# chinmay5/vit_ae_plus_plus

Measured on AMD Instinct MI355X. Metric: pretrain volumes/sec (96^3x4ch, mask 0.75) at 1/2/4/8 MI355X + recon-loss parity, higher is better.
Workload: dtype bf16; 1 GPU; ViT-B/16^3 contrastive MAE full optimisation step (fwd+loss+bwd+grad-norm+AdamW), synthetic BraTS-shape 96^3x4ch, batch 4/GPU, mask 0.75 (BASELINE config 2); global_batch=4, parallelism=dp1, rccl_ranks=1, hip_graph=True, weights=product initialize_weights, seed 0

## Files before the change

### vit_ae_plus_plus_amd/csrc/gemm_bt.hip

```cpp
#include "gemm_bt.hpp"

namespace vglds {

template <int BM, int BN, int WM, int WN, bool A_KC, bool B_KC>
__device__ __forceinline__ void gemm_bt_body(const GArgs& p, const int bid, const int zid, unsigned char* smem) {
    using Cf = BtCfg<BM, BN, WM, WN>;
    constexpr int NW = Cf::NW, HM = Cf::HM, HN = Cf::HN, FM = Cf::FM, FN = Cf::FN, NF = FM * FN;
    constexpr int A_HALF = Cf::A_HALF, B_HALF = Cf::B_HALF, BUF = Cf::BUF;
    constexpr bool STAGGER = NW == 8;
    constexpr int PA = pieces<HM, A_KC, NW>(), PB = pieces<HN, B_KC, NW>();
    constexpr int NACC = NF == 1 ? 2 : 1;
    constexpr bool ASM_READS = !A_KC || !B_KC;
    const int T = p.tiles_m * p.tiles_n;
    const int xq = T >> 3, xr = T & 7, xcd = bid & 7;
    const int lin = (xcd < xr ? xcd * (xq + 1) : xr * (xq + 1) + (xcd - xr) * xq) + (bid >> 3);
    if ((bid >> 3) >= xq + (xcd < xr ? 1 : 0)) return;
    const int tn = p.xcd_m ? lin % p.tiles_n : lin / p.tiles_m;
    const int tm = p.xcd_m ? lin / p.tiles_n : lin % p.tiles_m;
    const int m0 = tm * BM, n0 = tn * BN;
    const int kbeg = zid * p.k_per_split;
    const int nk = (min(p.K, kbeg + p.k_per_split) - kbeg) / BK;
    const int lane = threadIdx.x & 63;
    const int wave = __builtin_amdgcn_readfirstlane(threadIdx.x >> 6);
    const int wm = wave / WN, wn = wave % WN;
// ... 171 lines not shown
template <int BM, int BN, int WM, int WN>
static void bt_launch_cfg(const GArgs& p, bool a_kc, bool b_kc, hipStream_t st) {
    const dim3 grid(8 * cdiv((long)p.tiles_m * p.tiles_n, 8), 1, p.splits), block(64 * WM * WN);
    if (a_kc && b_kc) hipLaunchKernelGGL((gemm_bt_kernel<BM, BN, WM, WN, true, true>), grid, block, 0, st, p);
    else if (a_kc && !b_kc) hipLaunchKernelGGL((gemm_bt_kernel<BM, BN, WM, WN, true, false>), grid, block, 0, st, p);
    else if (!a_kc && !b_kc) hipLaunchKernelGGL((gemm_bt_kernel<BM, BN, WM, WN, false, false>), grid, block, 0, st, p);
}

bool bt_tile_dims(int id, int& bm, int& bn) {
    switch (id) {
        case 0: bm = 256; bn = 256; return true;
        case 3: bm = 128; bn = 128; return true;
        case 4: bm = 128; bn = 128; return true;
        case 5: bm = 64; bn = 64; return true;
        case 6: bm = 128; bn = 256; return true;
        default: return false;
    }
}

int bt_launch(GArgs p, int a_kc, int b_kc, int id, hipStream_t st) {
    int bm, bn;
    if (!bt_tile_dims(id, bm, bn)) return VITAE_ERR_INVALID_ARG;
    if (!p.vec_epi || p.a_rowsum || (p.K % BK) || p.splits < 1) return VITAE_ERR_UNSUPPORTED_SHAPE;
    if (!a_kc && b_kc) return VITAE_ERR_UNSUPPORTED_SHAPE;
    if (!bt_k_ranges(p.K, 2, p.splits, p.k_per_split)) return VITAE_ERR_UNSUPPORTED_SHAPE;
    p.tiles_m = cdiv(p.M, bm); p.tiles_n = cdiv(p.N, bn);
    if (p.splits > 1 && (!p.ws || id == 0 || (long)p.tiles_m * p.tiles_n > VITAE_GLDS_TICKETS || p.epi == VITAE_EPI_GELU)) return VITAE_ERR_UNSUPPORTED_SHAPE;
    if (id == 6 && (a_kc || b_kc)) return VITAE_ERR_UNSUPPORTED_SHAPE;
    if (id == 0) bt_launch_cfg<256, 256, 2, 4>(p, a_kc, b_kc, st);
    else if (id == 4 || id == 6) ws_launch(p, a_kc, b_kc, id, st);
    else if (id == 5) ws64_launch(p, a_kc, b_kc, st);
    else bt_launch_cfg<128, 128, 2, 2>(p, a_kc, b_kc, st);
    return vitae_launch_status();
}

int bt_wgrad_group_launch(GArgs* ps, int n, int splits, hipStream_t st, int kind ) {
    if (n < 1 || n > 4) return VITAE_ERR_INVALID_ARG;
    BtGroup g;
    int total = 0, tiles = 0;
    const int K = ps[0].K;
    int kps;
    if (!bt_k_ranges(K, 2, splits, kps)) return VITAE_ERR_UNSUPPORTED_SHAPE;
    for (int i = 0; i < 4; ++i) {
        g.start[i] = total;
        if (i >= n) { g.p[i] = g.p[0]; continue; }
        GArgs& p = ps[i];
// ... 18 lines not shown
```

### vit_ae_plus_plus_amd/csrc/gemm_bt.hpp

```cpp
#pragma once
#include <cstdlib>
#include <type_traits>
#include "glds_gemm.hpp"

namespace vglds {

using K0 = std::integral_constant<int, 0>; using K1 = std::integral_constant<int, 1>;
using K2 = std::integral_constant<int, 2>; using K3 = std::integral_constant<int, 3>;

__device__ __forceinline__ void wg_barrier() {
    __builtin_amdgcn_sched_barrier(0);
    __builtin_amdgcn_s_barrier();
    __builtin_amdgcn_sched_barrier(0);
}


template <int S, int PT> __device__ __forceinline__ void wait_tiles(const int fly) {
    if (S >= 5 && fly >= 3) wait_vmcnt<(S >= 5 ? 3 : 1) * PT>();
    else if (S >= 4 && fly >= 2) wait_vmcnt<(S >= 4 ? 2 : 1) * PT>();
    else if (fly >= 1) wait_vmcnt<PT>();
    else wait_vmcnt<0>();
}

static inline bool bt_k_ranges(const int K, const int min_tiles, int& splits, int& kps) {
// ... 372 lines not shown
        __builtin_amdgcn_sched_barrier(0);
        asm volatile("s_waitcnt lgkmcnt(0)" ::: "memory");
        if (t + 1 < nk) {
            wg_barrier();
            stage = stage + 1 == S ? 0 : stage + 1;
            const unsigned char* TN = smem + stage * STG;
            rd(TN, K0{}); rd(TN, K1{});
            __builtin_amdgcn_sched_barrier(0);
        }
        mm(K2{}); mm(K3{});
    }
}

void ws_launch(const GArgs& p, int a_kc, int b_kc, int id , hipStream_t st);
void ws_wgrad_group_launch(const BtGroup& g, int total, int splits, int kind , hipStream_t st);
void ws64_launch(const GArgs& p, int a_kc, int b_kc, hipStream_t st);

}
```

### vit_ae_plus_plus_amd/csrc/gemm_glds.hip

```cpp
#include <cstdlib>
#include "common.hpp"
#include "glds_tiles.hpp"
#include "glds_gemm.hpp"
#include "vitae_hip.h"

namespace {

using namespace vglds;

long long* g_gemm_dbg = nullptr;
double* g_wgrad_sqacc = nullptr;
int g_wgrad_sq_mask = 0, g_wgrad_sq_stride = 0;
static inline void set_sq(vglds::GArgs& p) { p.sqacc = g_wgrad_sqacc; p.sq_mask = g_wgrad_sq_mask; p.sq_stride = g_wgrad_sq_stride; }

struct EpiPre { f32x4 bias, res[4]; bool have; };

template <int BM, int BN, int NW>
__device__ __forceinline__ void epilogue_prefetch(const GArgs& p, int m0, int n0, EpiPre& e) {
    constexpr int NT = 64 * NW, CG = BN / 4, RPP = NT / CG, PASSES = BM / RPP;
    e.have = false;
    if constexpr (BM == 64 && BN == 64 && NW == 4) {
        static_assert(PASSES == 4, "prefetch geometry");
        if (!p.vec_epi) return;
        e.have = true;
// ... 528 lines not shown
    const int nkt = K / BK;
    static const int ws_on = getenv("VITAE_BT_WS") ? atoi(getenv("VITAE_BT_WS")) : 1;
    static const double ws_kt = getenv("VITAE_BT_WS_KT") ? atof(getenv("VITAE_BT_WS_KT")) : 800.0;
    static const int ws_min_rows = getenv("VITAE_BT_WS_MIN_ROWS") ? atoi(getenv("VITAE_BT_WS_MIN_ROWS")) : 2048;
    static const int ws_min_rows_fwd = getenv("VITAE_BT_WS_MIN_ROWS_FWD") ? atoi(getenv("VITAE_BT_WS_MIN_ROWS_FWD")) : 800;
    static const int ws_long_k = getenv("VITAE_BT_WS_LONG_K") ? atoi(getenv("VITAE_BT_WS_LONG_K")) : 8192;
    static const double ws_kt_w = getenv("VITAE_BT_WS_KT_W") ? atof(getenv("VITAE_BT_WS_KT_W")) : 900.0;
    static const double ws_fix = getenv("VITAE_BT_WS_FIX") ? atof(getenv("VITAE_BT_WS_FIX")) : 14000.0;
    static const int ws64_on = getenv("VITAE_BT_WS64") ? atoi(getenv("VITAE_BT_WS64")) : 1;
    static const double ws64_kt_w = getenv("VITAE_BT_WS64_KT_W") ? atof(getenv("VITAE_BT_WS64_KT_W")) : 650.0;
    static const int ws_long_any = getenv("VITAE_BT_WS_LONG_ANY") ? atoi(getenv("VITAE_BT_WS_LONG_ANY")) : 1;
    static const double bt_fix0 = getenv("VITAE_BT_FIX0") ? atof(getenv("VITAE_BT_FIX0")) : 9000.0;
    static const double bt_fix1 = getenv("VITAE_BT_FIX1") ? atof(getenv("VITAE_BT_FIX1")) : 4000.0;
    static const double wsw_kt = getenv("VITAE_BT_WSW_KT") ? atof(getenv("VITAE_BT_WSW_KT")) : 1350.0;
    static const int wsw_on = getenv("VITAE_BT_WSW") ? atoi(getenv("VITAE_BT_WSW")) : 1;
    for (int id : {0, 3, 4, 5, 6}) {
        if (only >= 0 && id != only) continue;
        if (id == 6 && (a_kc || b_kc || (g_bt_mode < 0 && !wsw_on))) continue;
        if (id == 5 && g_bt_mode != 5 && (!ws64_on || !allow_ws64)) continue;
        if (g_bt_mode >= 0 && id != g_bt_mode) continue;
        if (id == 4 && g_bt_mode < 0 && !ws_on) continue;
        if (id == 4 && g_bt_mode < 0 && (a_kc ? M : K) < ((a_kc && b_kc) ? ws_min_rows_fwd : ws_min_rows) && !(K >= ws_long_k && (ws_long_any || (a_kc ? M : K) < 1024))) continue;
        if (id == 6 && g_bt_mode < 0 && K < ws_min_rows && K < ws_long_k && (long)M * N < (1L << 22)) continue;
        int bm, bn;
        bt_tile_dims(id, bm, bn);
        const bool forced = g_bt_mode >= 0;
        if (!forced && (M < bm / 2 || N < bn / 2)) continue;
        const long tiles = (long)cdiv(M, bm) * cdiv(N, bn);
        static const int fsplit = getenv("VITAE_BT_SPLIT") ? atoi(getenv("VITAE_BT_SPLIT")) : 0;
        for (int s = 1; s <= (id >= 3 && allow_split ? (id == 6 ? 4 : 8) : 1); ++s) {
            if (forced && fsplit > 0 && s != fsplit) continue;
            const int kps = cdiv(cdiv(K, s), BK) * BK;
            if (cdiv(K, kps) != s || kps < (forced ? 2 : 4) * BK || K - (s - 1) * kps < 2 * BK) continue;
            if (s > 1 && (tiles > VITAE_GLDS_TICKETS || (cap >= 0 && VITAE_GLDS_TICKETS + tiles * s * bm * bn > cap))) continue;
            const double wgs = (double)tiles * s, slots = id == 3 ? 512 : 256;
            const double rounds = (double)cdiv((long)wgs, (long)slots);
            const double nk = (double)nkt / s;
            const double per = id == 0 ? 3000 + ((!a_kc && !b_kc) ? 4300 : 2950) * nk + 14500
                             : id == 6 ? ws_fix + 4000 + wsw_kt * nk + (s > 1 ? 9000 + 4000 * s : 0)
                             : id == 4 ? ws_fix + ((!a_kc && !b_kc) ? ws_kt_w : ws_kt) * nk + (s > 1 ? 6000 + 2200 * s : 0)
                                       : 4500 + 1800 * nk + 7500 + (s > 1 ? bt_fix0 + bt_fix1 * s : 0);
            double clk = rounds * per;
            if (id == 5) {
                const double over = wgs > 256 ? (wgs - 256) / 256 : 0, kt64 = (!a_kc && !b_kc && wgs >= 512) ? ws64_kt_w : 420;
                const double lat = (6500 + kt64 * nk + (s > 1 ? 3000 + 1000 * s : 0)) * (1 + 0.2 * over), thr = wgs * (3000 + kt64 * nk) / 256;
                clk = lat > thr ? lat : thr;
                if (nkt >= 128) clk *= 1.25;
            }
            if (clk < best.clocks) best = BtPlan{id, s, clk};
        }
    }
    if (best.tile < 0 || g_bt_mode >= 0 || only >= 0) return best;
    if (best.clocks >= 0.92 * est_64row(M, N, K, allow_split, !a_kc && !b_kc) * (nkt >= 128 ? 1.25 : 1.0)) return BtPlan{-1, 1, 0.0};
    return best;
}

template <int BM1, int BN1>
void launch_pair(int id2, dim3 grid, hipStream_t st, const GArgs& p1, const GArgs& p2, int nb1) {
    dim3 block(256);
    if (id2 == 0) hipLaunchKernelGGL((gemm_glds_pair_kernel<BM1, BN1, 64, 64>), grid, block, 0, st, p1, p2, nb1);
    else hipLaunchKernelGGL((gemm_glds_pair_kernel<BM1, BN1, 64, 128>), grid, block, 0, st, p1, p2, nb1);
}

}

extern "C" int vitae_gemm_glds_set_bt_tile(int mode) {
    if (mode < -2 || mode > 6 || mode == 1 || mode == 2) return VITAE_ERR_INVALID_ARG;
    g_bt_mode = mode;
    return VITAE_OK;
}

extern "C" int vitae_gemm_glds_bt_choice(int a_kcontig, int b_kcontig, int M, int N, int K) { return bt_plan(M, N, K, a_kcontig, b_kcontig, true).tile; }

extern "C" int vitae_gemm_glds_pick_split_k(int M, int N, int K) {
    const BtPlan bp = bt_plan(M, N, K, 1, 1, true);
    if (bp.tile >= 0) return bp.split;
    return old_split_rule(M, N, K);
}

extern "C" int vitae_gemm_glds_pick_split_k_form(int a_kcontig, int b_kcontig, int M, int N, int K) {
    const BtPlan bp = bt_plan(M, N, K, a_kcontig, b_kcontig, true);
    if (bp.tile >= 0) return bp.split;
// ... 36 lines not shown
    p.C = C; p.ldc = ldc; p.C16 = reinterpret_cast<__bf16*>(C16); p.ldc16 = ldc16;
    p.M = M; p.N = N; p.K = K;
    int kps = cdiv(cdiv(K, split_k), BK) * BK;
    split_k = cdiv(K, kps);
    if (split_k > 1 && !splitk_ws) return VITAE_ERR_INVALID_ARG;
    p.k_per_split = kps; p.splits = split_k;
    p.bias = bias; p.residual = residual; p.ldr = ldr; p.aux = aux; p.ldaux = ldaux;
    p.epi = epi; p.aux16 = aux16; p.auxd = auxd; p.accumulate = accumulate; p.ws = splitk_ws; p.out_colsum = out_colsum_accum; p.a_rowsum = nullptr;
    p.dbg = g_gemm_dbg;
    const Tile t = pick_tile(M, N);
    p.tiles_m = cdiv(M, t.bm); p.tiles_n = cdiv(N, t.bn);
    p.xcd_m = xcd_by_rows(M, N);
    p.vec_epi = vec_epilogue_ok(p);
    if (!a_kcontig && !b_kcontig) set_sq(p);
    if (p.vec_epi) {
        const BtPlan bp = forced ? *forced : bt_plan(M, N, K, a_kcontig, b_kcontig, epi != VITAE_EPI_GELU);
        if (bp.tile >= 0 && bp.split == split_k) {
            p.splits = split_k;
            return bt_launch(p, a_kcontig, b_kcontig, bp.tile, (hipStream_t)stream);
        }
    }
    if (split_k > 1 && (long)p.tiles_m * p.tiles_n > VITAE_GLDS_TICKETS) return VITAE_ERR_UNSUPPORTED_SHAPE;
    dim3 grid(glds_blocks(p), 1, split_k);
    hipStream_t st = (hipStream_t)stream;
    static const int pipe_max = getenv("VITAE_GLDS_PIPE_MAX_WGS") ? atoi(getenv("VITAE_GLDS_PIPE_MAX_WGS")) : 512;
    if (t.id == 0 && a_kcontig && b_kcontig && (long)grid.x * split_k <= pipe_max) {
        hipLaunchKernelGGL(gemm_glds_pipe_kernel, grid, dim3(256), 0, st, p);
        return vitae_launch_status();
    }
    if (t.id == 1) launch<64, 128>(p, a_kcontig != 0, b_kcontig != 0, grid, st);
    else launch<64, 64>(p, a_kcontig != 0, b_kcontig != 0, grid, st);
// ... 121 lines not shown
    const int epi_flags = (aux16 ? VITAE_EPI_AUX_BF16 : 0) | (auxd ? VITAE_EPI_AUX_DERIV : 0);
    if (dx_accumulate && !dx) return VITAE_ERR_INVALID_ARG;
    if ((N % BK) || (Mpad % BK) || (K & 7) || Mpad < M) return VITAE_ERR_UNSUPPORTED_SHAPE;
    if ((long)(M > N ? M : N) * K >= (1L << 31)) return VITAE_ERR_UNSUPPORTED_SHAPE;
    if ((long)Mpad * N >= (1L << 30) || (long)Mpad * K >= (1L << 30) || (long)N * K >= (1L << 30)) return VITAE_ERR_UNSUPPORTED_SHAPE;
    const long cap = splitk_ws && splitk_ws_floats > 0 ? splitk_ws_floats : 0;
    if (split_k > 1 && vitae_gemm_glds_ws_floats(M, K, split_k) > cap) return VITAE_ERR_INVALID_ARG;
    if (((uintptr_t)dy16 & 15) || ((uintptr_t)w16 & 15) || ((uintptr_t)x16 & 15)) return VITAE_ERR_UNSUPPORTED_SHAPE;
    if (!dw) {
        const BtPlan pd = bt_plan(M, K, N, 1, 0, true, cap);
        int sp = pd.tile >= 0 ? pd.split : old_split_rule(M, K, N);
        while (pd.tile < 0 && sp > 1 && vitae_gemm_glds_ws_floats(M, K, sp) > cap) --sp;
        return gemm_glds_launch(1, 0, dy16, N, w16, K, dx, K, dx16, K, M, K, N, nullptr, nullptr, 0, epi | epi_flags,
                                aux, K, dx_accumulate, sp, splitk_ws, dx_colsum_accum, stream, &pd);
    }
    auto ws64_pair = [&](int split) -> int {
        GArgs p1, p2;
        p1.A = reinterpret_cast<const __bf16*>(dy16); p1.lda = N;
        p1.B = reinterpret_cast<const __bf16*>(w16); p1.ldb = K;
        p1.C = dx; p1.ldc = K; p1.C16 = reinterpret_cast<__bf16*>(dx16); p1.ldc16 = K;
        p1.M = M; p1.N = K; p1.K = N; p1.k_per_split = N; p1.splits = split;
        p1.bias = nullptr; p1.residual = nullptr; p1.ldr = 0; p1.aux = aux; p1.ldaux = K; p1.epi = epi; p1.aux16 = aux16; p1.auxd = auxd;
        p1.accumulate = dx_accumulate != 0; p1.ws = splitk_ws; p1.out_colsum = dx_colsum_accum; p1.a_rowsum = nullptr; p1.dbg = g_gemm_dbg;
        p1.xcd_m = xcd_by_rows(M, K); p1.tiles_m = 0; p1.tiles_n = 0;
        p1.vec_epi = vec_epilogue_ok(p1);
        p2.A = reinterpret_cast<const __bf16*>(dy16); p2.lda = N;
        p2.B = reinterpret_cast<const __bf16*>(x16); p2.ldb = K;
        p2.C = dw; p2.ldc = K; p2.C16 = reinterpret_cast<__bf16*>(dw16); p2.ldc16 = K;
        p2.M = N; p2.N = K; p2.K = Mpad; p2.k_per_split = Mpad; p2.splits = 1;
        p2.bias = nullptr; p2.residual = nullptr; p2.ldr = 0; p2.aux = nullptr; p2.ldaux = 0; p2.epi = VITAE_EPI_NONE;
        p2.accumulate = dw_accumulate; p2.ws = nullptr; p2.out_colsum = nullptr; p2.a_rowsum = dy_colsum_accum; p2.dbg = g_gemm_dbg;
        set_sq(p2);
        p2.xcd_m = xcd_by_rows(N, K); p2.tiles_m = 0; p2.tiles_n = 0;
        p2.vec_epi = vec_epilogue_ok(p2);
        if (!p1.vec_epi || !p2.vec_epi) return VITAE_ERR_UNSUPPORTED_SHAPE;
        const char* wsq_env = getenv("VITAE_WS64Q");
        const int wsq = wsq_env ? atoi(wsq_env) : 0;
        const int rc = wsq ? ws64q_pair_launch(p1, p2, (hipStream_t)stream) : VITAE_ERR_UNSUPPORTED_SHAPE;
        return rc != VITAE_ERR_UNSUPPORTED_SHAPE ? rc : ws64_pair_launch(p1, p2, (hipStream_t)stream);
    };
    if (g_bt_mode == -1 || g_bt_mode == 5) {
        const BtPlan pd = bt_plan(M, K, N, 1, 0, true, cap), pw = bt_plan(N, K, Mpad, 0, 0, false, cap);
        if (pd.tile == 5 && pw.tile == 5) {
            const int rc = ws64_pair(pd.split);
            if (rc != VITAE_ERR_UNSUPPORTED_SHAPE) return rc;
        }
    }
    if (g_bt_mode != -2) {
        const BtPlan pd = bt_plan(M, K, N, 1, 0, true, cap, false), pw = bt_plan(N, K, Mpad, 0, 0, true, cap, false);
        if (pd.tile >= 0 || pw.tile >= 0) {
            auto fit = [&](const BtPlan& bp, int m, int n, int k) {
                if (bp.tile >= 0) return bp.split;
                int sp = old_split_rule(m, n, k);
                while (sp > 1 && vitae_gemm_glds_ws_floats(m, n, sp) > cap) --sp;
                return sp;
            };
            int rc = gemm_glds_launch(1, 0, dy16, N, w16, K, dx, K, dx16, K, M, K, N, nullptr, nullptr, 0, epi | epi_flags,
                                      aux, K, dx_accumulate, fit(pd, M, K, N), splitk_ws, dx_colsum_accum, stream, &pd);
            if (rc != VITAE_OK) return rc;
// ... 135 lines not shown
```

### vit_ae_plus_plus_amd/csrc/gemm_ws64.hip

```cpp
#include "gemm_bt.hpp"

namespace vglds {

#ifndef VITAE_WS64_STAGES
#define VITAE_WS64_STAGES 4
#endif
constexpr int WS64_SMEM = VITAE_WS64_STAGES * 16384;
template <bool A_KC, bool B_KC, int S, bool RS, bool W2 = false>
__device__ __forceinline__ void gemm_ws64_body(const GArgs& p, const WsHot& h, const int bid, const int zid, unsigned char* smem) {
#ifndef VITAE_WS64_PRODUCERS
#define VITAE_WS64_PRODUCERS 4
#endif
    constexpr int BM = 64, BN = 64, NWC = 4, NWP = VITAE_WS64_PRODUCERS;
    constexpr int A_T = BM * BK * 2, B_T = BN * BK * 2, STG = A_T + (W2 ? 2 : 1) * B_T;
    constexpr int PA = pieces<BM, A_KC, NWP>(), PB = pieces<BN, B_KC, NWP>(), PT = PA + (W2 ? 2 : 1) * PB;
    static_assert(!W2 || (A_KC && B_KC && !RS), "two weight planes: the forward form");
    static_assert(S >= 3 && S <= 5 && (S - 2) * PT <= 63, "stage count");
    const int T = h.tiles_m * h.tiles_n;
    const int xq = T >> 3, xr = T & 7, xcd = bid & 7;
    const int lin = (xcd < xr ? xcd * (xq + 1) : xr * (xq + 1) + (xcd - xr) * xq) + (bid >> 3);
    if ((bid >> 3) >= xq + (xcd < xr ? 1 : 0)) return;
    const int tn = (h.xcd_m & 1) ? lin % h.tiles_n : lin / h.tiles_m;
    const int tm = (h.xcd_m & 1) ? lin / h.tiles_n : lin % h.tiles_m;
    const int m0 = tm * BM, n0 = tn * BN;
    const int kbeg = zid * h.kps;
    const int nk = (min(h.K, kbeg + h.kps) - kbeg) / BK;
    const int lane = threadIdx.x & 63;
    const int wave = __builtin_amdgcn_readfirstlane(threadIdx.x >> 6);
// ... 36 lines not shown
    }
    const int wm = wave >> 1, wn = wave & 1;
    const int l31 = lane & 31, hi = lane >> 5;
    f32x16 acc[2];
#pragma unroll
    for (int h = 0; h < 2; ++h)
#pragma unroll
        for (int i = 0; i < 16; ++i) acc[h][i] = 0.f;
    const bool rowsum = RS && p.a_rowsum != nullptr && tn == 0 && wn == 0;
    f32x16 accx;
#pragma unroll
    for (int i = 0; i < 16; ++i) accx[i] = 0.f;
    bf16x8 ones;
#pragma unroll
    for (int i = 0; i < 8; ++i) ones[i] = (__bf16)1.0f;
    bf16x8 fa[BK / 16], fb[BK / 16], fb2[W2 ? BK / 16 : 1];
    constexpr int RK = (A_KC ? 1 : 2) + (W2 ? 2 : 1) * (B_KC ? 1 : 2);
    auto rd = [&](const unsigned char* TA, auto kk_c) {
        constexpr int kk = decltype(kk_c)::value;
        fa[kk] = frag_asm<BM, A_KC>(TA, wm * 32, kk, lane);
        fb[kk] = frag_asm<BN, B_KC>(TA + A_T, wn * 32, kk, lane);
        if constexpr (W2) fb2[kk] = frag_asm<BN, B_KC>(TA + A_T + B_T, wn * 32, kk, lane);
    };
    auto mm = [&](auto kk_c) {
        constexpr int kk = decltype(kk_c)::value;
        frag_tie(fa[kk]); frag_tie(fb[kk]);
        if constexpr (W2) {
            frag_tie(fb2[kk]);
            acc[kk & 1] = __builtin_amdgcn_mfma_f32_32x32x16_bf16(fa[kk], fb2[kk], acc[kk & 1], 0, 0, 0);
        }
        acc[kk & 1] = __builtin_amdgcn_mfma_f32_32x32x16_bf16(fa[kk], fb[kk], acc[kk & 1], 0, 0, 0);
        if constexpr (RS) {
            if (rowsum) accx = __builtin_amdgcn_mfma_f32_32x32x16_bf16(fa[kk], ones, accx, 0, 0, 0);
        }
    };
    const int nq = n0 + wn * 32 + 4 * (lane % 8);
    f32x4 bias4 = {0.f, 0.f, 0.f, 0.f};
    if (p.bias && nq < p.N) bias4 = *reinterpret_cast<const f32x4*>(p.bias + nq);
    stamp(0);
    wg_barrier();
    stamp(1);
    ws64_consume<2 * RK, S, STG>(smem, nk, rd, mm);
    if (RS && rowsum && l31 == 0) {
#pragma unroll
        for (int r = 0; r < 16; ++r) {
            const int m = m0 + wm * 32 + crow(r, hi);
            if (m < p.M) atomicAdd(p.a_rowsum + m, accx[r]);
        }
    }
    stamp(2);
    f32x16 accs[1][1];
#pragma unroll
    for (int i = 0; i < 16; ++i) accs[0][0][i] = acc[0][i] + acc[1][i];
    __syncthreads();
    float* Tw = reinterpret_cast<float*>(smem) + wave * 1024;
    if (p.splits > 1) {
        const int tile = p.tile0 + tm * p.tiles_n + tn;
        float* part = p.ws + VITAE_GLDS_TICKETS + (long)tile * p.splits * (BM * BN);
        const __amdgpu_buffer_rsrc_t rs = __builtin_amdgcn_make_buffer_rsrc(part, 0, p.splits * (BM * BN * 4), 0x00020000);
        typedef unsigned u32x4 __attribute__((ext_vector_type(4)));
        const int toff = (int)threadIdx.x * 16;
#pragma unroll
        for (int g = 0; g < 4; ++g) {
            const f32x4 v = {accs[0][0][4 * g], accs[0][0][4 * g + 1], accs[0][0][4 * g + 2], accs[0][0][4 * g + 3]};
            __builtin_amdgcn_raw_buffer_store_b128(__builtin_bit_cast(u32x4, v), rs, (zid * 4 + g) * (256 * 16) + toff, 0, 16);
        }
        asm volatile("s_waitcnt vmcnt(0)" ::: "memory");
        __syncthreads();
        int* flag = reinterpret_cast<int*>(smem + 4 * 4096);
        if (threadIdx.x == 0) *flag = __hip_atomic_fetch_add(reinterpret_cast<int*>(p.ws) + tile, 1, __ATOMIC_RELAXED, __HIP_MEMORY_SCOPE_AGENT);
        __syncthreads();
        stamp(3);
        if (*flag != p.splits - 1) return;
#pragma unroll
        for (int i = 0; i < 16; ++i) accs[0][0][i] = 0.f;
#pragma unroll 1
        for (int sp0 = 0; sp0 < p.splits; sp0 += 4) {
            f32x4 v[4][4];
#pragma unroll
            for (int u = 0; u < 4; ++u) {
                const int sp = min(sp0 + u, p.splits - 1);
#pragma unroll
                for (int g = 0; g < 4; ++g)
                    v[u][g] = __builtin_bit_cast(f32x4, __builtin_amdgcn_raw_buffer_load_b128(rs, (sp * 4 + g) * (256 * 16) + toff, 0, 16));
            }
#pragma unroll
            for (int u = 0; u < 4; ++u)
                if (sp0 + u < p.splits) {
#pragma unroll
                    for (int g = 0; g < 4; ++g)
#pragma unroll
                        for (int e = 0; e < 4; ++e) accs[0][0][4 * g + e] += v[u][g][e];
                }
        }
        if (threadIdx.x == 0) __hip_atomic_store(reinterpret_cast<int*>(p.ws) + tile, 0, __ATOMIC_RELAXED, __HIP_MEMORY_SCOPE_AGENT);
    }
    stamp(4);
    bt_park_quadrant<1, 1, 1>(accs, lane, Tw);
    __builtin_amdgcn_wave_barrier();
    float sqs = 0.f;
    { f32x4 cz = {0.f, 0.f, 0.f, 0.f}; bt_wave_epilogue<1, 1>(p, bt_epilogue_kind(p), m0 + wm * 32, n0 + wn * 32, Tw, lane, sqs, bias4, cz, false); }
    stamp(5);
    if (p.sqacc) {
        sqs = wave_sum(sqs);
        float* red = reinterpret_cast<float*>(smem + 4 * 4096 + 64);
        if (lane == 0) red[wave] = sqs;
        __syncthreads();
        if (threadIdx.x == 0) atomicAdd(sq_slot(p), (double)((red[0] + red[1]) + (red[2] + red[3])));
    }
    if (p.dbg) { asm volatile("s_waitcnt vmcnt(0)" ::: "memory"); stamp(6); }
}

template <bool A_KC, bool B_KC>
__global__ __launch_bounds__(64 * (4 + VITAE_WS64_PRODUCERS), 2) void gemm_ws64_kernel(WS_HOT_PARAMS, const GArgs p) {
    __shared__ __attribute__((aligned(1024))) unsigned char smem[WS64_SMEM];
    const WsHot h = WS_HOT_FROM_PARAMS;
    gemm_ws64_body<A_KC, B_KC, VITAE_WS64_STAGES, false>(p, h, blockIdx.x, blockIdx.z, smem);
}

void ws64_launch(const GArgs& p, int a_kc, int b_kc, hipStream_t st) {
    const dim3 grid(8 * cdiv((long)p.tiles_m * p.tiles_n, 8), 1, p.splits), block(64 * (4 + VITAE_WS64_PRODUCERS));
    if (a_kc && b_kc) hipLaunchKernelGGL((gemm_ws64_kernel<true, true>), grid, block, 0, st, WS_HOT_ARGS(p), p);
    else if (a_kc && !b_kc) hipLaunchKernelGGL((gemm_ws64_kernel<true, false>), grid, block, 0, st, WS_HOT_ARGS(p), p);
    else hipLaunchKernelGGL((gemm_ws64_kernel<false, false>), grid, block, 0, st, WS_HOT_ARGS(p), p);
}

constexpr int WS64W2_STAGES = 3;
__global__ __launch_bounds__(64 * (4 + VITAE_WS64_PRODUCERS), 2) void gemm_ws64_w2_kernel(WS_HOT_PARAMS, const GArgs p) {
    __shared__ __attribute__((aligned(1024))) unsigned char smem[WS64W2_STAGES * 24576];
    gemm_ws64_body<true, true, WS64W2_STAGES, false, true>(p, WS_HOT_FROM_PARAMS, blockIdx.x, blockIdx.z, smem);
}

int ws64_w2_launch(GArgs p, hipStream_t st) {
    if (!p.vec_epi || !p.B2 || p.a_rowsum || (p.K % BK) || p.splits < 1) return VITAE_ERR_UNSUPPORTED_SHAPE;
    if (!bt_k_ranges(p.K, 2, p.splits, p.k_per_split)) return VITAE_ERR_UNSUPPORTED_SHAPE;
    p.tiles_m = cdiv(p.M, 64); p.tiles_n = cdiv(p.N, 64); p.tile0 = 0;
    if (p.splits > 1 && (!p.ws || (long)p.tiles_m * p.tiles_n > VITAE_GLDS_TICKETS || p.epi == VITAE_EPI_GELU)) return VITAE_ERR_UNSUPPORTED_SHAPE;
    const dim3 grid(8 * cdiv((long)p.tiles_m * p.tiles_n, 8), 1, p.splits), block(64 * (4 + VITAE_WS64_PRODUCERS));
    hipLaunchKernelGGL(gemm_ws64_w2_kernel, grid, block, 0, st, WS_HOT_ARGS(p), p);
    return vitae_launch_status();
}

template <bool RS>
__global__ __launch_bounds__(64 * (4 + VITAE_WS64_PRODUCERS), 2) void gemm_ws64_pair_kernel(const __bf16* A, const __bf16* B1, const __bf16* B2, int lda, int ldb,
                                                                                           int M1, int N1, int K1, int K2, int kps1, int packed,
                                                                                           const GArgs p1, const GArgs p2) {
    __shared__ __attribute__((aligned(1024))) unsigned char smem[WS64_SMEM];
    const int nb1 = packed & 0xfffff, splits1 = (packed >> 20) & 15, dbg2 = (packed >> 25) & 2;
    if ((int)blockIdx.x < nb1 * splits1) {
        const WsHot h{A, B1, nullptr, lda, ldb, M1, N1, K1, (M1 + 63) >> 6, (N1 + 63) >> 6, ((packed >> 24) & 1) | dbg2, kps1};
        gemm_ws64_body<true, false, VITAE_WS64_STAGES, false>(p1, h, blockIdx.x % nb1, blockIdx.x / nb1, smem);
    } else {
        const WsHot h{A, B2, nullptr, lda, ldb, K1, N1, K2, (K1 + 63) >> 6, (N1 + 63) >> 6, ((packed >> 25) & 1) | dbg2, K2};
        gemm_ws64_body<false, false, VITAE_WS64_STAGES, RS>(p2, h, blockIdx.x - nb1 * splits1, 0, smem);
    }
}

int ws64_pair_launch(GArgs p1, GArgs p2, hipStream_t st) {
    if (!p1.vec_epi || !p2.vec_epi || (p1.K % BK) || (p2.K % BK) || p2.K < 2 * BK || p1.a_rowsum) return VITAE_ERR_UNSUPPORTED_SHAPE;
    if (p1.splits < 1) p1.splits = 1;
    if (!bt_k_ranges(p1.K, 2, p1.splits, p1.k_per_split)) return VITAE_ERR_UNSUPPORTED_SHAPE;
    p1.tiles_m = cdiv(p1.M, 64); p1.tiles_n = cdiv(p1.N, 64); p1.tile0 = 0;
    p2.tiles_m = cdiv(p2.M, 64); p2.tiles_n = cdiv(p2.N, 64); p2.tile0 = 0;
    p2.k_per_split = p2.K; p2.splits = 1;
    if (p1.splits > 1 && (!p1.ws || (long)p1.tiles_m * p1.tiles_n > VITAE_GLDS_TICKETS)) return VITAE_ERR_UNSUPPORTED_SHAPE;
    const int nb1 = 8 * cdiv((long)p1.tiles_m * p1.tiles_n, 8), nb2 = 8 * cdiv((long)p2.tiles_m * p2.tiles_n, 8);
    const dim3 grid(nb1 * p1.splits + nb2), block(64 * (4 + VITAE_WS64_PRODUCERS));
    if (p1.A != p2.A || p1.lda != p2.lda || p1.ldb != p2.ldb || p2.M != p1.K || p2.N != p1.N || nb1 >= (1 << 20) || p1.splits > 15 ||
        p1.lda >= (1L << 31) || p1.ldb >= (1L << 31)) return VITAE_ERR_UNSUPPORTED_SHAPE;
    const int packed = nb1 | p1.splits << 20 | (p1.xcd_m & 1) << 24 | (p2.xcd_m & 1) << 25 | ((p1.dbg || p2.dbg) ? 1 << 26 : 0);
    if (p2.a_rowsum) hipLaunchKernelGGL((gemm_ws64_pair_kernel<true>), grid, block, 0, st, p1.A, p1.B, p2.B, (int)p1.lda, (int)p1.ldb, p1.M, p1.N, p1.K,
                                        p2.K, p1.k_per_split, packed, p1, p2);
    else hipLaunchKernelGGL((gemm_ws64_pair_kernel<false>), grid, block, 0, st, p1.A, p1.B, p2.B, (int)p1.lda, (int)p1.ldb, p1.M, p1.N, p1.K,
                            p2.K, p1.k_per_split, packed, p1, p2);
    return vitae_launch_status();
}

}
```

### vit_ae_plus_plus_amd/csrc/glds_gemm.hpp

```cpp
#pragma once
#include "common.hpp"
#include "glds_tiles.hpp"
#include "vitae_hip.h"

namespace vglds {

struct GArgs {
    const __bf16* A; long lda;
    const __bf16* B; long ldb;
    float* C; long ldc;
    __bf16* C16; long ldc16;
    int M, N, K;
    int k_per_split, splits;
    const float* bias;
    const float* residual; long ldr;
    float* aux; long ldaux;
    int epi, accumulate;
    float* ws;
    float* out_colsum;
    float* a_rowsum;
    int vec_epi;
    int tiles_m, tiles_n;
    double* sqacc = nullptr;
    int sq_mask = 0, sq_stride = 0;
// ... 64 lines not shown
                if (acc_c) x += co[q];
                p.C[m * ldc + n] = x;
            }
            if (p.C16) p.C16[m * ldc16 + n] = (__bf16)x;
            csum += x;
            sqsum += x * x;
        }
        asm volatile("" ::: "memory");
    }
    return csum;
}

bool bt_tile_dims(int id, int& bm, int& bn);
int bt_launch(GArgs p, int a_kc, int b_kc, int id, hipStream_t st);
int bt_wgrad_group_launch(GArgs* ps, int n, int splits, hipStream_t st, int kind);
int ws64_pair_launch(GArgs p1, GArgs p2, hipStream_t st);
int ws64q_pair_launch(GArgs p1, GArgs p2, hipStream_t st);
int wsx3_launch(GArgs p, int a_kc, int b_kc, hipStream_t st);
int ws64_w2_launch(GArgs p, hipStream_t st);
int wsx3_slots();

}
```

Before: 1145 volumes/s.

## Add 128x64 warp-specialized tile variant and use it in backward dgrad/wgrad pair

Generalizes the warp-specialized 64x64 GEMM body to a 128-row tile (two A fragments sharing one B fragment, three pipeline stages) and adds it as tile id 7. By default, the fused backward dgrad+wgrad pair kernel switches to 128-row tiles when the tile count is high and the reduction depth is short. The aim is more MFMA work per B-fragment load and fewer workgroups, cutting LDS and global traffic per flop. In exchange the kernel uses more registers and shared memory and has fewer stages, which may hurt latency hiding or occupancy.

```diff
diff --git a/vit_ae_plus_plus_amd/csrc/gemm_bt.hip b/vit_ae_plus_plus_amd/csrc/gemm_bt.hip
--- a/vit_ae_plus_plus_amd/csrc/gemm_bt.hip
+++ b/vit_ae_plus_plus_amd/csrc/gemm_bt.hip
@@ -209,6 +209,7 @@
         case 4: bm = 128; bn = 128; return true;
         case 5: bm = 64; bn = 64; return true;
         case 6: bm = 128; bn = 256; return true;
+        case 7: bm = 128; bn = 64; return true;
         default: return false;
     }
 }
@@ -224,7 +225,7 @@
     if (id == 6 && (a_kc || b_kc)) return VITAE_ERR_UNSUPPORTED_SHAPE;
     if (id == 0) bt_launch_cfg<256, 256, 2, 4>(p, a_kc, b_kc, st);
     else if (id == 4 || id == 6) ws_launch(p, a_kc, b_kc, id, st);
-    else if (id == 5) ws64_launch(p, a_kc, b_kc, st);
+    else if (id == 5 || id == 7) ws64_launch(p, a_kc, b_kc, id, st);
     else bt_launch_cfg<128, 128, 2, 2>(p, a_kc, b_kc, st);
     return vitae_launch_status();
 }
diff --git a/vit_ae_plus_plus_amd/csrc/gemm_bt.hpp b/vit_ae_plus_plus_amd/csrc/gemm_bt.hpp
--- a/vit_ae_plus_plus_amd/csrc/gemm_bt.hpp
+++ b/vit_ae_plus_plus_amd/csrc/gemm_bt.hpp
@@ -410,6 +410,6 @@
 
 void ws_launch(const GArgs& p, int a_kc, int b_kc, int id , hipStream_t st);
 void ws_wgrad_group_launch(const BtGroup& g, int total, int splits, int kind , hipStream_t st);
-void ws64_launch(const GArgs& p, int a_kc, int b_kc, hipStream_t st);
-
-}
+void ws64_launch(const GArgs& p, int a_kc, int b_kc, int id , hipStream_t st);
+
+}
diff --git a/vit_ae_plus_plus_amd/csrc/gemm_glds.hip b/vit_ae_plus_plus_amd/csrc/gemm_glds.hip
--- a/vit_ae_plus_plus_amd/csrc/gemm_glds.hip
+++ b/vit_ae_plus_plus_amd/csrc/gemm_glds.hip
@@ -566,8 +566,9 @@
     static const double bt_fix1 = getenv("VITAE_BT_FIX1") ? atof(getenv("VITAE_BT_FIX1")) : 4000.0;
     static const double wsw_kt = getenv("VITAE_BT_WSW_KT") ? atof(getenv("VITAE_BT_WSW_KT")) : 1350.0;
     static const int wsw_on = getenv("VITAE_BT_WSW") ? atoi(getenv("VITAE_BT_WSW")) : 1;
-    for (int id : {0, 3, 4, 5, 6}) {
+    for (int id : {0, 3, 4, 5, 6, 7}) {
         if (only >= 0 && id != only) continue;
+        if (id == 7 && g_bt_mode != 7 && only != 7) continue;
         if (id == 6 && (a_kc || b_kc || (g_bt_mode < 0 && !wsw_on))) continue;
         if (id == 5 && g_bt_mode != 5 && (!ws64_on || !allow_ws64)) continue;
         if (g_bt_mode >= 0 && id != g_bt_mode) continue;
@@ -593,6 +594,12 @@
                              : id == 4 ? ws_fix + ((!a_kc && !b_kc) ? ws_kt_w : ws_kt) * nk + (s > 1 ? 6000 + 2200 * s : 0)
                                        : 4500 + 1800 * nk + 7500 + (s > 1 ? bt_fix0 + bt_fix1 * s : 0);
             double clk = rounds * per;
+            if (id == 7) {
+                const double over = wgs > 256 ? (wgs - 256) / 256 : 0, kt = ((!a_kc && !b_kc && wgs >= 512) ? ws64_kt_w : 420) * 1.5;
+                const double lat = (7500 + kt * nk + (s > 1 ? 3000 + 1000 * s : 0)) * (1 + 0.2 * over), thr = wgs * (4000 + kt * nk) / 256;
+                clk = lat > thr ? lat : thr;
+                if (nkt >= 128) clk *= 1.25;
+            }
             if (id == 5) {
                 const double over = wgs > 256 ? (wgs - 256) / 256 : 0, kt64 = (!a_kc && !b_kc && wgs >= 512) ? ws64_kt_w : 420;
                 const double lat = (6500 + kt64 * nk + (s > 1 ? 3000 + 1000 * s : 0)) * (1 + 0.2 * over), thr = wgs * (3000 + kt64 * nk) / 256;
@@ -617,7 +624,7 @@
 }
 
 extern "C" int vitae_gemm_glds_set_bt_tile(int mode) {
-    if (mode < -2 || mode > 6 || mode == 1 || mode == 2) return VITAE_ERR_INVALID_ARG;
+    if (mode < -2 || mode > 7 || mode == 1 || mode == 2) return VITAE_ERR_INVALID_ARG;
     g_bt_mode = mode;
     return VITAE_OK;
 }
@@ -684,7 +691,8 @@
     p.vec_epi = vec_epilogue_ok(p);
     if (!a_kcontig && !b_kcontig) set_sq(p);
     if (p.vec_epi) {
-        const BtPlan bp = forced ? *forced : bt_plan(M, N, K, a_kcontig, b_kcontig, epi != VITAE_EPI_GELU);
+        BtPlan bp = forced ? *forced : bt_plan(M, N, K, a_kcontig, b_kcontig, epi != VITAE_EPI_GELU);
+        if (!forced && g_bt_mode == 7 && bp.tile == 7) bp.split = split_k;
         if (bp.tile >= 0 && bp.split == split_k) {
             p.splits = split_k;
             return bt_launch(p, a_kcontig, b_kcontig, bp.tile, (hipStream_t)stream);
@@ -836,7 +844,7 @@
         return gemm_glds_launch(1, 0, dy16, N, w16, K, dx, K, dx16, K, M, K, N, nullptr, nullptr, 0, epi | epi_flags,
                                 aux, K, dx_accumulate, sp, splitk_ws, dx_colsum_accum, stream, &pd);
     }
-    auto ws64_pair = [&](int split) -> int {
+    auto ws64_pair = [&](int split, int bm1 = 64, int bm2 = 64) -> int {
         GArgs p1, p2;
         p1.A = reinterpret_cast<const __bf16*>(dy16); p1.lda = N;
         p1.B = reinterpret_cast<const __bf16*>(w16); p1.ldb = K;
@@ -858,13 +866,31 @@
         if (!p1.vec_epi || !p2.vec_epi) return VITAE_ERR_UNSUPPORTED_SHAPE;
         const char* wsq_env = getenv("VITAE_WS64Q");
         const int wsq = wsq_env ? atoi(wsq_env) : 0;
-        const int rc = wsq ? ws64q_pair_launch(p1, p2, (hipStream_t)stream) : VITAE_ERR_UNSUPPORTED_SHAPE;
-        return rc != VITAE_ERR_UNSUPPORTED_SHAPE ? rc : ws64_pair_launch(p1, p2, (hipStream_t)stream);
+        const int rc = (wsq && bm1 == 64 && bm2 == 64) ? ws64q_pair_launch(p1, p2, (hipStream_t)stream) : VITAE_ERR_UNSUPPORTED_SHAPE;
+        return rc != VITAE_ERR_UNSUPPORTED_SHAPE ? rc : ws64_pair_launch(p1, p2, (hipStream_t)stream, bm1, bm2);
     };
+    if (g_bt_mode == 7) {
+        const char* pt = getenv("VITAE_PAIR_TILES");
+        const int bm1 = (pt && pt[0] == '5') ? 64 : 128, bm2 = (pt && pt[0] && pt[1] == '5') ? 64 : 128;
+        const BtPlan pd = bt_plan(M, K, N, 1, 0, true, cap);
+        if (pd.tile == 7) {
+            const int rc = ws64_pair(pd.split, bm1, bm2);
+            if (rc != VITAE_ERR_UNSUPPORTED_SHAPE) return rc;
+        }
+    }
     if (g_bt_mode == -1 || g_bt_mode == 5) {
         const BtPlan pd = bt_plan(M, K, N, 1, 0, true, cap), pw = bt_plan(N, K, Mpad, 0, 0, false, cap);
         if (pd.tile == 5 && pw.tile == 5) {
-            const int rc = ws64_pair(pd.split);
+            static const int t7_on = getenv("VITAE_PAIR_T7") ? atoi(getenv("VITAE_PAIR_T7")) : 1;
+            int bm1 = 64, bm2 = 64;
+            if (g_bt_mode == -1 && t7_on && pd.split == 1) {
+                const long w5 = (long)cdiv(N, 64) * cdiv(K, 64), d5 = (long)cdiv(M, 64) * cdiv(K, 64);
+                if (N / BK <= 16 && d5 + (w5 >= 384 ? (long)cdiv(N, 128) * cdiv(K, 64) : w5) >= 448) {
+                    bm1 = 128;
+                    if (w5 >= 384) bm2 = 128;
+                }
+            }
+            const int rc = ws64_pair(pd.split, bm1, bm2);
             if (rc != VITAE_ERR_UNSUPPORTED_SHAPE) return rc;
         }
     }
diff --git a/vit_ae_plus_plus_amd/csrc/gemm_ws64.hip b/vit_ae_plus_plus_amd/csrc/gemm_ws64.hip
--- a/vit_ae_plus_plus_amd/csrc/gemm_ws64.hip
+++ b/vit_ae_plus_plus_amd/csrc/gemm_ws64.hip
@@ -6,12 +6,13 @@
 #define VITAE_WS64_STAGES 4
 #endif
 constexpr int WS64_SMEM = VITAE_WS64_STAGES * 16384;
-template <bool A_KC, bool B_KC, int S, bool RS, bool W2 = false>
+template <bool A_KC, bool B_KC, int S, bool RS, bool W2 = false, int BM = 64>
 __device__ __forceinline__ void gemm_ws64_body(const GArgs& p, const WsHot& h, const int bid, const int zid, unsigned char* smem) {
 #ifndef VITAE_WS64_PRODUCERS
 #define VITAE_WS64_PRODUCERS 4
 #endif
-    constexpr int BM = 64, BN = 64, NWC = 4, NWP = VITAE_WS64_PRODUCERS;
+    constexpr int BN = 64, NWC = 4, NWP = VITAE_WS64_PRODUCERS, FM = BM / 64;
+    static_assert(BM == 64 || (BM == 128 && !W2), "64 or 128 rows");
     constexpr int A_T = BM * BK * 2, B_T = BN * BK * 2, STG = A_T + (W2 ? 2 : 1) * B_T;
     constexpr int PA = pieces<BM, A_KC, NWP>(), PB = pieces<BN, B_KC, NWP>(), PT = PA + (W2 ? 2 : 1) * PB;
     static_assert(!W2 || (A_KC && B_KC && !RS), "two weight planes: the forward form");
@@ -78,24 +79,46 @@
     bf16x8 ones;
 #pragma unroll
     for (int i = 0; i < 8; ++i) ones[i] = (__bf16)1.0f;
-    bf16x8 fa[BK / 16], fb[BK / 16], fb2[W2 ? BK / 16 : 1];
-    constexpr int RK = (A_KC ? 1 : 2) + (W2 ? 2 : 1) * (B_KC ? 1 : 2);
+    bf16x8 fa[FM][BK / 16], fb[BK / 16], fb2[W2 ? BK / 16 : 1];
+    constexpr int RK = FM * (A_KC ? 1 : 2) + (W2 ? 2 : 1) * (B_KC ? 1 : 2);
+    static_assert(2 * RK <= 15, "the counted lgkmcnt of ws64_consume");
+    bf16x8 sel[2];
+    if constexpr (FM == 2 && RS) {
+#pragma unroll
+        for (int i = 0; i < 8; ++i) {
+            sel[0][i] = (__bf16)((lane & 16) ? 0.0f : 1.0f);
+            sel[1][i] = (__bf16)((lane & 16) ? 1.0f : 0.0f);
+        }
+    }
     auto rd = [&](const unsigned char* TA, auto kk_c) {
         constexpr int kk = decltype(kk_c)::value;
-        fa[kk] = frag_asm<BM, A_KC>(TA, wm * 32, kk, lane);
+        fa[0][kk] = frag_asm<BM, A_KC>(TA, wm * (BM / 2), kk, lane);
+        if constexpr (FM == 2) fa[1][kk] = frag_asm<BM, A_KC>(TA, wm * (BM / 2) + 32, kk, lane);
         fb[kk] = frag_asm<BN, B_KC>(TA + A_T, wn * 32, kk, lane);
         if constexpr (W2) fb2[kk] = frag_asm<BN, B_KC>(TA + A_T + B_T, wn * 32, kk, lane);
     };
     auto mm = [&](auto kk_c) {
         constexpr int kk = decltype(kk_c)::value;
-        frag_tie(fa[kk]); frag_tie(fb[kk]);
+        if constexpr (FM == 2) {
+            frag_tie(fa[0][kk]); frag_tie(fa[1][kk]); frag_tie(fb[kk]);
+            acc[0] = __builtin_amdgcn_mfma_f32_32x32x16_bf16(fa[0][kk], fb[kk], acc[0], 0, 0, 0);
+            acc[1] = __builtin_amdgcn_mfma_f32_32x32x16_bf16(fa[1][kk], fb[kk], acc[1], 0, 0, 0);
+            if constexpr (RS) {
+                if (rowsum) {
+                    accx = __builtin_amdgcn_mfma_f32_32x32x16_bf16(sel[0], fa[0][kk], accx, 0, 0, 0);
+                    accx = __builtin_amdgcn_mfma_f32_32x32x16_bf16(sel[1], fa[1][kk], accx, 0, 0, 0);
+                }
+            }
+            return;
+        }
+        frag_tie(fa[0][kk]); frag_tie(fb[kk]);
         if constexpr (W2) {
             frag_tie(fb2[kk]);
-            acc[kk & 1] = __builtin_amdgcn_mfma_f32_32x32x16_bf16(fa[kk], fb2[kk], acc[kk & 1], 0, 0, 0);
-        }
-        acc[kk & 1] = __builtin_amdgcn_mfma_f32_32x32x16_bf16(fa[kk], fb[kk], acc[kk & 1], 0, 0, 0);
+            acc[kk & 1] = __builtin_amdgcn_mfma_f32_32x32x16_bf16(fa[0][kk], fb2[kk], acc[kk & 1], 0, 0, 0);
+        }
+        acc[kk & 1] = __builtin_amdgcn_mfma_f32_32x32x16_bf16(fa[0][kk], fb[kk], acc[kk & 1], 0, 0, 0);
         if constexpr (RS) {
-            if (rowsum) accx = __builtin_amdgcn_mfma_f32_32x32x16_bf16(fa[kk], ones, accx, 0, 0, 0);
+            if (rowsum) accx = __builtin_amdgcn_mfma_f32_32x32x16_bf16(fa[0][kk], ones, accx, 0, 0, 0);
         }
     };
     const int nq = n0 + wn * 32 + 4 * (lane % 8);
@@ -105,7 +128,14 @@
     wg_barrier();
     stamp(1);
     ws64_consume<2 * RK, S, STG>(smem, nk, rd, mm);
-    if (RS && rowsum && l31 == 0) {
+    if constexpr (FM == 2) {
+        if (RS && rowsum && hi == 0) {
+            const int m = m0 + wm * 64 + l31;
+            if (m < p.M) atomicAdd(p.a_rowsum + m, accx[0]);
+            if (m + 32 < p.M) atomicAdd(p.a_rowsum + m + 32, accx[8]);
+        }
+    }
+    if (FM == 1 && RS && rowsum && l31 == 0) {
 #pragma unroll
         for (int r = 0; r < 16; ++r) {
             const int m = m0 + wm * 32 + crow(r, hi);
@@ -113,11 +143,15 @@
         }
     }
     stamp(2);
-    f32x16 accs[1][1];
-#pragma unroll
-    for (int i = 0; i < 16; ++i) accs[0][0][i] = acc[0][i] + acc[1][i];
+    f32x16 accs[1][FM];
+    if constexpr (FM == 2) {
+        accs[0][0] = acc[0]; accs[0][1] = acc[1];
+    } else {
+#pragma unroll
+        for (int i = 0; i < 16; ++i) accs[0][0][i] = acc[0][i] + acc[1][i];
+    }
     __syncthreads();
-    float* Tw = reinterpret_cast<float*>(smem) + wave * 1024;
+    float* Tw = reinterpret_cast<float*>(smem) + wave * (1024 * FM);
     if (p.splits > 1) {
         const int tile = p.tile0 + tm * p.tiles_n + tn;
         float* part = p.ws + VITAE_GLDS_TICKETS + (long)tile * p.splits * (BM * BN);
@@ -125,49 +159,52 @@
         typedef unsigned u32x4 __attribute__((ext_vector_type(4)));
         const int toff = (int)threadIdx.x * 16;
 #pragma unroll
-        for (int g = 0; g < 4; ++g) {
-            const f32x4 v = {accs[0][0][4 * g], accs[0][0][4 * g + 1], accs[0][0][4 * g + 2], accs[0][0][4 * g + 3]};
-            __builtin_amdgcn_raw_buffer_store_b128(__builtin_bit_cast(u32x4, v), rs, (zid * 4 + g) * (256 * 16) + toff, 0, 16);
+        for (int g = 0; g < 4 * FM; ++g) {
+            const f32x4 v = {accs[0][g >> 2][4 * (g & 3)], accs[0][g >> 2][4 * (g & 3) + 1], accs[0][g >> 2][4 * (g & 3) + 2], accs[0][g >> 2][4 * (g & 3) + 3]};
+            __builtin_amdgcn_raw_buffer_store_b128(__builtin_bit_cast(u32x4, v), rs, (zid * (4 * FM) + g) * (256 * 16) + toff, 0, 16);
         }
         asm volatile("s_waitcnt vmcnt(0)" ::: "memory");
         __syncthreads();
-        int* flag = reinterpret_cast<int*>(smem + 4 * 4096);
+        int* flag = reinterpret_cast<int*>(smem + 4 * 4096 * FM);
         if (threadIdx.x == 0) *flag = __hip_atomic_fetch_add(reinterpret_cast<int*>(p.ws) + tile, 1, __ATOMIC_RELAXED, __HIP_MEMORY_SCOPE_AGENT);
         __syncthreads();
         stamp(3);
         if (*flag != p.splits - 1) return;
 #pragma unroll
-        for (int i = 0; i < 16; ++i) accs[0][0][i] = 0.f;
+        for (int f = 0; f < FM; ++f)
+#pragma unroll
+            for (int i = 0; i < 16; ++i) accs[0][f][i] = 0.f;
+        constexpr int SU = 4 / FM;
 #pragma unroll 1
-        for (int sp0 = 0; sp0 < p.splits; sp0 += 4) {
-            f32x4 v[4][4];
-#pragma unroll
-            for (int u = 0; u < 4; ++u) {
+        for (int sp0 = 0; sp0 < p.splits; sp0 += SU) {
+            f32x4 v[SU][4 * FM];
+#pragma unroll
+            for (int u = 0; u < SU; ++u) {
                 const int sp = min(sp0 + u, p.splits - 1);
 #pragma unroll
-                for (int g = 0; g < 4; ++g)
-                    v[u][g] = __builtin_bit_cast(f32x4, __builtin_amdgcn_raw_buffer_load_b128(rs, (sp * 4 + g) * (256 * 16) + toff, 0, 16));
+                for (int g = 0; g < 4 * FM; ++g)
+                    v[u][g] = __builtin_bit_cast(f32x4, __builtin_amdgcn_raw_buffer_load_b128(rs, (sp * (4 * FM) + g) * (256 * 16) + toff, 0, 16));
             }
 #pragma unroll
-            for (int u = 0; u < 4; ++u)
+            for (int u = 0; u < SU; ++u)
                 if (sp0 + u < p.splits) {
 #pragma unroll
-                    for (int g = 0; g < 4; ++g)
-#pragma unroll
-                        for (int e = 0; e < 4; ++e) accs[0][0][4 * g + e] += v[u][g][e];
+                    for (int g = 0; g < 4 * FM; ++g)
+#pragma unroll
+                        for (int e = 0; e < 4; ++e) accs[0][g >> 2][4 * (g & 3) + e] += v[u][g][e];
                 }
         }
         if (threadIdx.x == 0) __hip_atomic_store(reinterpret_cast<int*>(p.ws) + tile, 0, __ATOMIC_RELAXED, __HIP_MEMORY_SCOPE_AGENT);
     }
     stamp(4);
-    bt_park_quadrant<1, 1, 1>(accs, lane, Tw);
+    bt_park_quadrant<FM, 1, 1>(accs, lane, Tw);
     __builtin_amdgcn_wave_barrier();
     float sqs = 0.f;
-    { f32x4 cz = {0.f, 0.f, 0.f, 0.f}; bt_wave_epilogue<1, 1>(p, bt_epilogue_kind(p), m0 + wm * 32, n0 + wn * 32, Tw, lane, sqs, bias4, cz, false); }
+    { f32x4 cz = {0.f, 0.f, 0.f, 0.f}; bt_wave_epilogue<FM, 1>(p, bt_epilogue_kind(p), m0 + wm * (BM / 2), n0 + wn * 32, Tw, lane, sqs, bias4, cz, false); }
     stamp(5);
     if (p.sqacc) {
         sqs = wave_sum(sqs);
-        float* red = reinterpret_cast<float*>(smem + 4 * 4096 + 64);
+        float* red = reinterpret_cast<float*>(smem + 4 * 4096 * FM + 64);
         if (lane == 0) red[wave] = sqs;
         __syncthreads();
         if (threadIdx.x == 0) atomicAdd(sq_slot(p), (double)((red[0] + red[1]) + (red[2] + red[3])));
@@ -182,8 +219,22 @@
     gemm_ws64_body<A_KC, B_KC, VITAE_WS64_STAGES, false>(p, h, blockIdx.x, blockIdx.z, smem);
 }
 
-void ws64_launch(const GArgs& p, int a_kc, int b_kc, hipStream_t st) {
+constexpr int WS128X64_STAGES = 3, WS128X64_SMEM = WS128X64_STAGES * 24576;
+template <bool A_KC, bool B_KC>
+__global__ __launch_bounds__(64 * (4 + VITAE_WS64_PRODUCERS), 2) void gemm_ws64_m128_kernel(WS_HOT_PARAMS, const GArgs p) {
+    __shared__ __attribute__((aligned(1024))) unsigned char smem[WS128X64_SMEM];
+    const WsHot h{A, B, B2, lda, ldb, M, N, K, (M + 127) >> 7, (N + 63) >> 6, xcd_m, kps};
+    gemm_ws64_body<A_KC, B_KC, WS128X64_STAGES, false, false, 128>(p, h, blockIdx.x, blockIdx.z, smem);
+}
+
+void ws64_launch(const GArgs& p, int a_kc, int b_kc, int id, hipStream_t st) {
     const dim3 grid(8 * cdiv((long)p.tiles_m * p.tiles_n, 8), 1, p.splits), block(64 * (4 + VITAE_WS64_PRODUCERS));
+    if (id == 7) {
+        if (a_kc && b_kc) hipLaunchKernelGGL((gemm_ws64_m128_kernel<true, true>), grid, block, 0, st, WS_HOT_ARGS(p), p);
+        else if (a_kc && !b_kc) hipLaunchKernelGGL((gemm_ws64_m128_kernel<true, false>), grid, block, 0, st, WS_HOT_ARGS(p), p);
+        else hipLaunchKernelGGL((gemm_ws64_m128_kernel<false, false>), grid, block, 0, st, WS_HOT_ARGS(p), p);
+        return;
+    }
     if (a_kc && b_kc) hipLaunchKernelGGL((gemm_ws64_kernel<true, true>), grid, block, 0, st, WS_HOT_ARGS(p), p);
     else if (a_kc && !b_kc) hipLaunchKernelGGL((gemm_ws64_kernel<true, false>), grid, block, 0, st, WS_HOT_ARGS(p), p);
     else hipLaunchKernelGGL((gemm_ws64_kernel<false, false>), grid, block, 0, st, WS_HOT_ARGS(p), p);
@@ -205,27 +256,43 @@
     return vitae_launch_status();
 }
 
-template <bool RS>
+template <bool RS, int BM1, int BM2>
 __global__ __launch_bounds__(64 * (4 + VITAE_WS64_PRODUCERS), 2) void gemm_ws64_pair_kernel(const __bf16* A, const __bf16* B1, const __bf16* B2, int lda, int ldb,
                                                                                            int M1, int N1, int K1, int K2, int kps1, int packed,
                                                                                            const GArgs p1, const GArgs p2) {
-    __shared__ __attribute__((aligned(1024))) unsigned char smem[WS64_SMEM];
+    constexpr int S1 = BM1 == 128 ? WS128X64_STAGES : VITAE_WS64_STAGES, S2 = BM2 == 128 ? WS128X64_STAGES : VITAE_WS64_STAGES;
+    constexpr int SMEM = (BM1 == 128 || BM2 == 128) ? WS128X64_SMEM : WS64_SMEM;
+    static_assert(SMEM >= WS64_SMEM && 2 * SMEM <= 160 * 1024, "either body's stages; two workgroups per CU");
+    __shared__ __attribute__((aligned(1024))) unsigned char smem[SMEM];
     const int nb1 = packed & 0xfffff, splits1 = (packed >> 20) & 15, dbg2 = (packed >> 25) & 2;
     if ((int)blockIdx.x < nb1 * splits1) {
-        const WsHot h{A, B1, nullptr, lda, ldb, M1, N1, K1, (M1 + 63) >> 6, (N1 + 63) >> 6, ((packed >> 24) & 1) | dbg2, kps1};
-        gemm_ws64_body<true, false, VITAE_WS64_STAGES, false>(p1, h, blockIdx.x % nb1, blockIdx.x / nb1, smem);
+        const WsHot h{A, B1, nullptr, lda, ldb, M1, N1, K1, (M1 + BM1 - 1) >> (BM1 == 128 ? 7 : 6), (N1 + 63) >> 6, ((packed >> 24) & 1) | dbg2, kps1};
+        gemm_ws64_body<true, false, S1, false, false, BM1>(p1, h, blockIdx.x % nb1, blockIdx.x / nb1, smem);
     } else {
-        const WsHot h{A, B2, nullptr, lda, ldb, K1, N1, K2, (K1 + 63) >> 6, (N1 + 63) >> 6, ((packed >> 25) & 1) | dbg2, K2};
-        gemm_ws64_body<false, false, VITAE_WS64_STAGES, RS>(p2, h, blockIdx.x - nb1 * splits1, 0, smem);
-    }
-}
-
-int ws64_pair_launch(GArgs p1, GArgs p2, hipStream_t st) {
+        const WsHot h{A, B2, nullptr, lda, ldb, K1, N1, K2, (K1 + BM2 - 1) >> (BM2 == 128 ? 7 : 6), (N1 + 63) >> 6, ((packed >> 25) & 1) | dbg2, K2};
+        gemm_ws64_body<false, false, S2, RS, false, BM2>(p2, h, blockIdx.x - nb1 * splits1, 0, smem);
+    }
+}
+
+template <bool RS>
+static void ws64_pair_dispatch(int bm1, int bm2, dim3 grid, dim3 block, hipStream_t st, const GArgs& p1, const GArgs& p2, int packed) {
+#define VITAE_WS64_PAIR(B1, B2)                                                                                                              \
+    hipLaunchKernelGGL((gemm_ws64_pair_kernel<RS, B1, B2>), grid, block, 0, st, p1.A, p1.B, p2.B, (int)p1.lda, (int)p1.ldb, p1.M, p1.N, p1.K, \
+                       p2.K, p1.k_per_split, packed, p1, p2)
+    if (bm1 == 64 && bm2 == 64) VITAE_WS64_PAIR(64, 64);
+    else if (bm1 == 64) VITAE_WS64_PAIR(64, 128);
+    else if (bm2 == 64) VITAE_WS64_PAIR(128, 64);
+    else VITAE_WS64_PAIR(128, 128);
+#undef VITAE_WS64_PAIR
+}
+
+int ws64_pair_launch(GArgs p1, GArgs p2, hipStream_t st, int bm1, int bm2) {
+    if ((bm1 != 64 && bm1 != 128) || (bm2 != 64 && bm2 != 128)) return VITAE_ERR_INVALID_ARG;
     if (!p1.vec_epi || !p2.vec_epi || (p1.K % BK) || (p2.K % BK) || p2.K < 2 * BK || p1.a_rowsum) return VITAE_ERR_UNSUPPORTED_SHAPE;
     if (p1.splits < 1) p1.splits = 1;
     if (!bt_k_ranges(p1.K, 2, p1.splits, p1.k_per_split)) return VITAE_ERR_UNSUPPORTED_SHAPE;
-    p1.tiles_m = cdiv(p1.M, 64); p1.tiles_n = cdiv(p1.N, 64); p1.tile0 = 0;
-    p2.tiles_m = cdiv(p2.M, 64); p2.tiles_n = cdiv(p2.N, 64); p2.tile0 = 0;
+    p1.tiles_m = cdiv(p1.M, bm1); p1.tiles_n = cdiv(p1.N, 64); p1.tile0 = 0;
+    p2.tiles_m = cdiv(p2.M, bm2); p2.tiles_n = cdiv(p2.N, 64); p2.tile0 = 0;
     p2.k_per_split = p2.K; p2.splits = 1;
     if (p1.splits > 1 && (!p1.ws || (long)p1.tiles_m * p1.tiles_n > VITAE_GLDS_TICKETS)) return VITAE_ERR_UNSUPPORTED_SHAPE;
     const int nb1 = 8 * cdiv((long)p1.tiles_m * p1.tiles_n, 8), nb2 = 8 * cdiv((long)p2.tiles_m * p2.tiles_n, 8);
@@ -233,10 +300,8 @@
     if (p1.A != p2.A || p1.lda != p2.lda || p1.ldb != p2.ldb || p2.M != p1.K || p2.N != p1.N || nb1 >= (1 << 20) || p1.splits > 15 ||
         p1.lda >= (1L << 31) || p1.ldb >= (1L << 31)) return VITAE_ERR_UNSUPPORTED_SHAPE;
     const int packed = nb1 | p1.splits << 20 | (p1.xcd_m & 1) << 24 | (p2.xcd_m & 1) << 25 | ((p1.dbg || p2.dbg) ? 1 << 26 : 0);
-    if (p2.a_rowsum) hipLaunchKernelGGL((gemm_ws64_pair_kernel<true>), grid, block, 0, st, p1.A, p1.B, p2.B, (int)p1.lda, (int)p1.ldb, p1.M, p1.N, p1.K,
-                                        p2.K, p1.k_per_split, packed, p1, p2);
-    else hipLaunchKernelGGL((gemm_ws64_pair_kernel<false>), grid, block, 0, st, p1.A, p1.B, p2.B, (int)p1.lda, (int)p1.ldb, p1.M, p1.N, p1.K,
-                            p2.K, p1.k_per_split, packed, p1, p2);
+    if (p2.a_rowsum) ws64_pair_dispatch<true>(bm1, bm2, grid, block, st, p1, p2, packed);
+    else ws64_pair_dispatch<false>(bm1, bm2, grid, block, st, p1, p2, packed);
     return vitae_launch_status();
 }
 
diff --git a/vit_ae_plus_plus_amd/csrc/glds_gemm.hpp b/vit_ae_plus_plus_amd/csrc/glds_gemm.hpp
--- a/vit_ae_plus_plus_amd/csrc/glds_gemm.hpp
+++ b/vit_ae_plus_plus_amd/csrc/glds_gemm.hpp
@@ -102,7 +102,7 @@
 bool bt_tile_dims(int id, int& bm, int& bn);
 int bt_launch(GArgs p, int a_kc, int b_kc, int id, hipStream_t st);
 int bt_wgrad_group_launch(GArgs* ps, int n, int splits, hipStream_t st, int kind);
-int ws64_pair_launch(GArgs p1, GArgs p2, hipStream_t st);
+int ws64_pair_launch(GArgs p1, GArgs p2, hipStream_t st, int bm1 = 64, int bm2 = 64);
 int ws64q_pair_launch(GArgs p1, GArgs p2, hipStream_t st);
 int wsx3_launch(GArgs p, int a_kc, int b_kc, hipStream_t st);
 int ws64_w2_launch(GArgs p, hipStream_t st);
```

Result: faster. 1159 volumes/s (median of 6 runs) (+1.2%).
